# AlexandraLJones/MCBRaT3D

Measured on AMD Instinct MI355X. Metric: photons/sec, higher is better.
Workload: dtype f32/f64

## Files before the change

mcbrat3d_amd/csrc/mcbrat_api.hip:

```cpp
#include <hip/hip_runtime.h>

#include <algorithm>
#include <array>
#include <cfloat>
#include <cmath>
#include <cstdio>
#include <cstdlib>
#include <cstring>
#include <string>
#include <vector>

#include "mcbrat_kernels.hip"
#include "mcbrat_blockwalk.hip"

using namespace mcbrat;

struct mcbrat_ctx {
  int device = 0;
  struct Lane {
    hipStream_t stream = nullptr;
    hipEvent_t ev0 = nullptr, ev1 = nullptr;
    hipEvent_t evDone = nullptr;
    unsigned long long *dCounter = nullptr;
    long long *dSlabs = nullptr;
// ... 33 lines not shown
  uint16_t *dFlyRange = nullptr;
  int flyNbx = 0, flyNby = 0;
  bool flyBuilt = false;
  double flyDepth = 0.0;
  double flightMaxDepth = 0.5;
  uint32_t *dBlockRec = nullptr;
  uint16_t *dBlockOf = nullptr;
  float *dBlockExt = nullptr;
  float *dBlockSsa = nullptr, *dBlockCum = nullptr;
  uint16_t *dBlockPfi = nullptr;
  bool blockOpticsUniform = false;
  int nBlocks = 0;
  int crossThreshold = 8;
  int batchUnits = 0;
  int jumpThreshold = 8;
  bool noSimple3 = false;
  float *dExtB = nullptr, *dCumB = nullptr, *dSsaB = nullptr, *dBgExt = nullptr, *dBgCum = nullptr, *dBgSsa = nullptr;
  uint16_t *dPfiB = nullptr, *dBgPfi = nullptr;
  int nbx = 0, nby = 0, nbz = 0;
  long long nStored = 0;
  double backgroundFraction = 0.0;
  bool bricksBuilt = false;
  int brickMode = 2;
  float *dTables = nullptr;
  int surfNumX = 0, surfNumY = 0;
  double *dSurfX = nullptr, *dSurfY = nullptr;
  float *dSurfRefl = nullptr;
  int surfKind = 0;
  float4 *dSurfBrdf = nullptr;
  double *dVoxelCDF = nullptr;
// ... 392 lines not shown
  return 0;
}

int build_blocks(mcbrat_ctx *c, const std::vector<float> &e, const std::vector<float> &cu, const std::vector<float> &ssa,
                 const std::vector<uint16_t> &pf, int nc) {
  const int nx = c->nx, ny = c->ny, nz = c->nz;
  const size_t nvox = (size_t)nx * ny * nz;
  c->nBlocks = 0;
  if (c->dBlockRec) { (void)hipFree(c->dBlockRec); c->dBlockRec = nullptr; }
  if (c->dBlockOf) { (void)hipFree(c->dBlockOf); c->dBlockOf = nullptr; }
  if (c->dBlockExt) { (void)hipFree(c->dBlockExt); c->dBlockExt = nullptr; }
  if (c->dBlockSsa) { (void)hipFree(c->dBlockSsa); c->dBlockSsa = nullptr; }
  if (c->dBlockCum) { (void)hipFree(c->dBlockCum); c->dBlockCum = nullptr; }
  if (c->dBlockPfi) { (void)hipFree(c->dBlockPfi); c->dBlockPfi = nullptr; }
  c->blockOpticsUniform = false;
  if (nvox > 65536 || nx > 65535 || ny > 65535 || nz > 65535) return 0;
  std::vector<uint16_t> of(nvox);
  std::vector<uint32_t> rec(4 * nvox);
  int32_t nb = 0;
  if (mcbrat_block_decomposition(nx, ny, nz, e.data(), of.data(), rec.data(), &nb) != 0) return 0;
  std::vector<float> blockExt((size_t)nb, 0.0f);
  for (size_t v = 0; v < nvox; ++v) blockExt[of[v]] = e[v];
  if (upload(c, &c->dBlockRec, rec.data(), (size_t)4 * nb) || upload(c, &c->dBlockOf, of.data(), of.size()) ||
      upload(c, &c->dBlockExt, blockExt.data(), blockExt.size())) return 1;
  std::vector<float> bSsa((size_t)nc * nb), bCum((size_t)nc * nb);
  std::vector<uint16_t> bPfi((size_t)nc * nb);
  std::vector<char> seen((size_t)nb, 0);
  bool uniform = true;
  for (size_t v = 0; v < nvox && uniform; ++v) {
    const size_t b = of[v];
    for (int k = 0; k < nc && uniform; ++k) {
      const size_t i = (size_t)k * nvox + v, j = (size_t)k * nb + b;
      if (!seen[b]) { bSsa[j] = ssa[i]; bCum[j] = cu[i]; bPfi[j] = pf[i]; }
      else uniform = std::memcmp(&bSsa[j], &ssa[i], 4) == 0 && std::memcmp(&bCum[j], &cu[i], 4) == 0 && bPfi[j] == pf[i];
    }
    seen[b] = 1;
  }
  if (uniform) {
    if (upload(c, &c->dBlockSsa, bSsa.data(), bSsa.size()) || upload(c, &c->dBlockCum, bCum.data(), bCum.size()) ||
        upload(c, &c->dBlockPfi, bPfi.data(), bPfi.size())) return 1;
    c->blockOpticsUniform = true;
  }
  c->nBlocks = nb;
  return 0;
}

bool use_bricks(const mcbrat_ctx *c) {
  if (!c->bricksBuilt || c->brickMode == 0 || c->nDir > 0 || orders_on(c) || facewalk_on(c)) return false;
  if (c->brickMode == 1) return true;
  const size_t nvox = (size_t)c->nx * c->ny * c->nz;
  return nvox * sizeof(float) >= ((size_t)2 << 30) && c->backgroundFraction >= 0.5;
}

void fill_params(mcbrat_ctx *c, DevParams &p) {
  std::memset(&p, 0, sizeof(p));
  p.nx = c->nx; p.ny = c->ny; p.nz = c->nz; p.nc = c->nc;
  p.xyRegular = c->xyRegular; p.zRegular = c->zRegular;
// ... 315 lines not shown
        MCBRAT_SPEC_CASE(1 | 1 << 2 | 16); MCBRAT_SPEC_CASE(2 | 1 << 2 | 16); MCBRAT_SPEC_CASE(3 | 1 << 2 | 16);
        MCBRAT_SPEC_CASE(1 | 2 << 2 | 16); MCBRAT_SPEC_CASE(2 | 2 << 2 | 16); MCBRAT_SPEC_CASE(3 | 2 << 2 | 16);
#undef MCBRAT_SPEC_CASE
      }
    }
  }
  return trace_ptr<BLOCK, 0, false, DBG>(tbl, emit);
}

template <int BLOCK, bool DBG, int SIMPLE, int OPT>
const void *block_ptr(bool tbl, bool emit) {
  if (tbl) return emit ? (const void *)trace_block_kernel<BLOCK, true, DBG, true, SIMPLE, OPT> : (const void *)trace_block_kernel<BLOCK, true, DBG, false, SIMPLE, OPT>;
  return emit ? (const void *)trace_block_kernel<BLOCK, false, DBG, true, SIMPLE, OPT> : (const void *)trace_block_kernel<BLOCK, false, DBG, false, SIMPLE, OPT>;
}

template <int BLOCK, bool DBG, int OPT = 0>
const void *block_kernel_for(const mcbrat_ctx *c, const DevParams &p, bool tbl) {
  const bool emit = c->srcKind != 0;
  const bool simple = c->xyRegular && c->zRegular && c->nc == 1 && c->surfNumX == 0;
  if constexpr (OPT == 0 && BLOCK != 1024) {
    if (simple && c->ny == 1 && !DBG) return block_ptr<BLOCK, DBG, 2, OPT>(tbl, emit);
  }
  if constexpr (!DBG && (BLOCK == 1024 || BLOCK == 768)) {
    if (!c->xyRegular && !c->zRegular && p.xyNearUniform && p.zNearUniform && c->nc == 1 && c->surfNumX == 0 && !c->noSimple3)
      return block_ptr<BLOCK, DBG, 3, OPT>(tbl, emit);
  }
  return simple ? block_ptr<BLOCK, DBG, 1, OPT>(tbl, emit) : block_ptr<BLOCK, DBG, 0, OPT>(tbl, emit);
}

bool block_walk_applies(const mcbrat_ctx *c, const LaunchPlan &L) {
  return blocks_worth_it(c) && ((L.priv && L.gridLds) || L.blockLite);
}

int launch_block(mcbrat_ctx *c, DevParams &p, const LaunchPlan &L, bool debug, int nBatches) {
// ... 781 lines not shown
             kernel == 2 ? "trace_block_kernel" : "trace_kernel", h[3], kind == DROP_RAY ? "view direction" : "state", state, (unsigned)(h[2] >> 32));
  } else {
    snprintf(buf + at, sizeof(buf) - (size_t)at, "; no photon record (production kernels keep none: trace the same photons with mcbrat_trace_fates)");
  }
  c->dropText = buf;
  return c->dropText.c_str();
}

int mcbrat_set_option(mcbrat_ctx *c, const char *name, int32_t value) {
  if (!c) return 1;
  if (!name) return fail(c, "set_option: no option name");
  const std::string n(name);
  if (n == "jumpThreshold") c->jumpThreshold = std::max(1, std::min(64, (int)value));
  else if (n == "crossThreshold") c->crossThreshold = std::max(1, std::min(64, (int)value));
  else if (n == "batchUnits") c->batchUnits = value != 0;
  else return fail(c, "set_option: unknown option '" + n + "'");
  return 0;
}

int mcbrat_set_surface_description(mcbrat_ctx *c, int32_t numX, int32_t numY, const double *xPosition, const double *yPosition,
                                   const float *reflectance) {
  if (!c) return 1;
  (void)hipSetDevice(c->device);
  if (sync_all(c)) return 1;
  if (numX <= 0 || numY <= 0) { c->surfNumX = c->surfNumY = 0; return 0; }
  if (numX < 2 || numY < 2 || !xPosition || !yPosition || !reflectance)
    return fail(c, "new_SurfaceDescription: position vector(s) are incorrect length.");
  for (int i = 1; i < numX; ++i) if (!(xPosition[i] - xPosition[i - 1] > 0.)) return fail(c, "new_SurfaceDescription: positions must be unique, increasing.");
  for (int i = 1; i < numY; ++i) if (!(yPosition[i] - yPosition[i - 1] > 0.)) return fail(c, "new_SurfaceDescription: positions must be unique, increasing.");
  for (size_t i = 0; i < (size_t)(numX - 1) * (numY - 1); ++i)
// ... 111 lines not shown
  if (e == hipSuccess) e = hipMemcpyAsync(out, dOut, sizeof(uint32_t) * 4 * (size_t)n, hipMemcpyDeviceToHost, st);
  if (e == hipSuccess) e = hipStreamSynchronize(st);
  (void)hipFree(dIn); (void)hipFree(dOut);
  HIP_OK(c, e);
  return 0;
}

int mcbrat_get_walk_mode(const mcbrat_ctx *c) {
  if (!c) return 0;
  int m = (c->layerSkip ? 1 : 0) | (c->blockWalk ? 2 : 0);
  if (c->haveGrid && c->haveOptics) {
    const LaunchPlan L = plan_launch(c, (size_t)tally_layout(flux_run(tally_shape(c))).slabStride);
    m = ((c->layerSkip && !facewalk_on(c)) ? 1 : 0) | (block_walk_applies(c, L) ? 2 : 0) | (L.fly ? 4 : 0) | (c->blockWalk ? 8 : 0) |
        (L.wide ? 16 : 0) | ((L.blockLite && L.optics == 1) ? 32 : 0) | (L.priv ? 64 : 0) | ((L.blockLite && L.optics == 2) ? 128 : 0) |
        (L.cdfTop ? 256 : 0);
  }
  return m;
}

int mcbrat_compute_radiative_transfer(mcbrat_ctx *c, uint64_t seed, uint64_t firstPhotonId, int64_t ppb, int32_t nBatches,
                                      int64_t *numPhotonsProcessed) {
  if (!c) return 1;
  (void)hipSetDevice(c->device);
  if (check_ready(c)) return 1;
  if (ppb < 1 || nBatches < 1) return fail(c, "computeRadiativeTransfer: Didn't process any photons.");
  if (ppb > kMaxPhotonsPerBatch)
    return fail(c, "computeRadiativeTransfer: numPhotonsPerBatch is too large: at most 2^31 - 1 photons per batch fit the tallies.");
  if (ensure_moments(c)) return 1;
  const bool tuneNow = c->autoTune && !c->tuned && (unsigned long long)ppb * (unsigned long long)nBatches >= c->tuneTrialPhotons;
  const bool async = c->asyncOn && !c->countersOn;
// ... 250 lines not shown
```

mcbrat3d_amd/csrc/mcbrat_blockwalk.hip:

```cpp
#include <float.h>

#include "mcbrat_device.h"

namespace mcbrat {

enum : int { BW_DEAD = 0, BW_MOVE = 1, BW_COLLIDE = 2, BW_SURFACE = 3, BW_TOP = 4, BW_CROSS = 5 };

__device__ __forceinline__ int locate_z(const double *ze, int nz, bool regular, double z0, double invDz, double z) {
  if (!regular) return find_cell(ze, nz, z);
  return min(max((int)((z - z0) * invDz), 0), nz - 1);
}
__device__ __forceinline__ int locate_near_uniform(const double *e, int n, double x0, double invCell, double v) {
  int i = min(max((int)((v - x0) * invCell), 0), n - 1);
  const double lo = e[i], hi = e[i + 1];
  i += (v >= hi && i < n - 1) ? 1 : 0;
  i -= (v < lo && i > 0) ? 1 : 0;
  return i;
}

__device__ __forceinline__ long long unwrapped_index(const double *e, int n, double x0, double L, double invL, double x) {
  const double k = floor((x - x0) * invL);
  return (long long)k * n + find_cell(e, n, x - k * L);
}

struct BlockLds {
  size_t slab, cursor, rec, cdf, ext, ssa, cum, pfi, blockOf, tbl, total;
};
__host__ __device__ inline BlockLds block_lds_layout(int nx, int ny, int nz, int nc, size_t slabLen, int nBlocks, size_t tblFloats,
                                                      int optics = 0, bool cdfTop = false) {
  BlockLds L;
  const size_t nvox = (size_t)nx * ny * nz;
  const size_t nB4 = ((size_t)nBlocks + 3) & ~(size_t)3;
  size_t o = sizeof(double) * (size_t)(nx + ny + nz + 3);
  L.slab = o; o += sizeof(long long) * slabLen;
  L.cursor = o; o += 16;
  o = (o + 15) & ~(size_t)15;
  L.rec = o; o += 16 * (size_t)nBlocks;
  L.cdf = o; o += cdfTop ? sizeof(double) * ((size_t)nz + (size_t)ny * nz) : 0;
  L.ext = o; o += optics == 0 ? 4 * nvox : 4 * nB4;
  L.ssa = o; o += optics == 0 ? 4 * nvox * nc : (optics == 2 ? 4 * nB4 * nc : 0);
  L.cum = o; o += nc > 1 ? (optics == 0 ? 4 * nvox * nc : (optics == 2 ? 4 * nB4 * nc : 0)) : 0;
  L.pfi = o; o += optics == 0 ? 2 * ((nvox * nc + 1) & ~(size_t)1) : (optics == 2 ? 2 * nB4 * nc : 0);
  L.blockOf = o; o += 2 * ((nvox + 1) & ~(size_t)1);
  o = (o + 3) & ~(size_t)3;
  L.tbl = o; o += 4 * tblFloats;
  L.total = o;
  return L;
}

template <int BLOCK, bool TBL_LDS, bool DEBUG, bool EMIT, int SIMPLE, int OPT = 0>
__global__ void __launch_bounds__(BLOCK, BLOCK == 1024 ? 4 : (BLOCK > 512 ? BLOCK / 128 : MCBRAT_MIN_WAVES_PER_SIMD))
trace_block_kernel(const DevParams p) {
  constexpr bool NOY = SIMPLE == 2 && !DEBUG;
  constexpr bool NEAR = SIMPLE == 3;
  const bool xyRegular = NEAR ? false : (SIMPLE != 0 ? true : p.xyRegular != 0);
  const bool zRegular = NEAR ? false : (SIMPLE != 0 ? true : p.zRegular != 0);
  const int nc = SIMPLE != 0 ? 1 : p.nc;
  extern __shared__ __align__(16) unsigned char smem_raw[];
#ifdef MCBRAT_POISON
  for (unsigned i = threadIdx.x; i < p.ldsBytes / 4u; i += BLOCK) reinterpret_cast<unsigned *>(smem_raw)[i] = 0xffffffffu;
  __syncthreads();
#endif
  double *s_edge = reinterpret_cast<double *>(smem_raw);
  const int nEdges = p.nx + p.ny + p.nz + 3;
  const int ncol = p.nx * p.ny;
  const int nvox = ncol * p.nz;
  const int slabLen = (int)p.slabStride;
  const int slabsLen = p.unitsWide ? 2 * slabLen : slabLen;
  const bool cdfTop = EMIT && p.cdfTopLds != 0;
  const BlockLds lay = block_lds_layout(p.nx, p.ny, p.nz, nc, (size_t)slabsLen, p.nBlocks, TBL_LDS ? (size_t)p.tblTotalFloats : 0, OPT, cdfTop);
  const int nB4 = (p.nBlocks + 3) & ~3;
  long long *s_slab = reinterpret_cast<long long *>(smem_raw + lay.slab);
  unsigned *s_cursor = reinterpret_cast<unsigned *>(smem_raw + lay.cursor);
  uint4 *s_blockRec = reinterpret_cast<uint4 *>(smem_raw + lay.rec);
  float *s_ext = reinterpret_cast<float *>(smem_raw + lay.ext);
  double *s_cdfLevel = reinterpret_cast<double *>(smem_raw + lay.cdf);
  double *s_cdfRow = s_cdfLevel + p.nz;
  float *s_ssa = reinterpret_cast<float *>(smem_raw + lay.ssa);
  float *s_cum = reinterpret_cast<float *>(smem_raw + lay.cum);
  uint16_t *s_pfi = reinterpret_cast<uint16_t *>(smem_raw + lay.pfi);
  uint16_t *s_blockOf = reinterpret_cast<uint16_t *>(smem_raw + lay.blockOf);
  float *s_tbl = reinterpret_cast<float *>(smem_raw + lay.tbl);
  __shared__ int s_tblOffset[MCBRAT_MAX_COMPONENTS], s_tblNSteps[MCBRAT_MAX_COMPONENTS];
  __shared__ float s_tblInvN[MCBRAT_MAX_COMPONENTS];
  if (threadIdx.x < MCBRAT_MAX_COMPONENTS) {
    s_tblOffset[threadIdx.x] = p.tblOffset[threadIdx.x];
    s_tblNSteps[threadIdx.x] = p.tblNSteps[threadIdx.x];
    s_tblInvN[threadIdx.x] = p.tblInvN[threadIdx.x];
  }
  for (int i = threadIdx.x; i < nEdges; i += BLOCK) s_edge[i] = p.edges[i];
  if (TBL_LDS)
    for (int i = threadIdx.x; i < p.tblTotalFloats; i += BLOCK) s_tbl[i] = p.tables[i];
  for (int i = threadIdx.x; i < slabsLen; i += BLOCK) s_slab[i] = 0;
  if (threadIdx.x == 0) s_cursor[0] = 0;
  for (int i = threadIdx.x; i < p.nBlocks; i += BLOCK) s_blockRec[i] = p.blockRec[i];
  for (int i = threadIdx.x; i < nvox; i += BLOCK) s_blockOf[i] = p.blockOf[i];
  if (OPT == 0) {
    for (int i = threadIdx.x; i < nvox; i += BLOCK) s_ext[i] = p.ext[i];
    for (int i = threadIdx.x; i < nc * nvox; i += BLOCK) { s_ssa[i] = p.ssa[i]; s_pfi[i] = p.pfi[i]; }
    if (nc > 1)
      for (int i = threadIdx.x; i < nc * nvox; i += BLOCK) s_cum[i] = p.cum[i];
  } else {
    for (int i = threadIdx.x; i < p.nBlocks; i += BLOCK) s_ext[i] = p.blockExt[i];
    if (OPT == 2) {
      for (int i = threadIdx.x; i < nc * nB4; i += BLOCK) {
        const int k = i / nB4, b = i - k * nB4;
        if (b < p.nBlocks) { s_ssa[i] = p.blockSsa[k * p.nBlocks + b]; s_pfi[i] = p.blockPfi[k * p.nBlocks + b]; if (nc > 1) s_cum[i] = p.blockCum[k * p.nBlocks + b]; }
      }
    }
  }
// ... 9 lines not shown
  auto extOfCell = [&](int cell) -> float { if constexpr (OPT == 0) return s_ext[cell]; else return s_ext[s_blockOf[cell]]; };
  const float *__restrict__ tbl = TBL_LDS ? s_tbl : p.tables;
  const int offY = p.nx + 1, offZ = p.nx + p.ny + 2;
  const double invDz = (double)p.nz / (p.zMax - p.z0);

  const int lane = threadIdx.x & (kWave - 1);

  unsigned long long unitFirst = 0;
  unsigned unitCount = 0, unitSplit = 0;
  long long *unitSlab = nullptr;

  int state = BW_DEAD;
  unsigned long long moreMask = ~0ull;
  int slabOff = 0;
  uint32_t idLo = 0, idHi = 0, event = 0;
  unsigned long long idP1 = 0;
  double px = 0, py = 0, pz = 0;
  float dx = 0, dy = 0, dz = 1;
  float ivx = 0, ivy = 0, ivz = 0;
  float tnx = 0, tny = 0, tnz = 0, tcur = 0;
  float acc = 0, tau = 0, w = 0, extCur = 0, uX = 0, uY = 0, uZ = 0;
  unsigned rx = 0, ry = 0, rz = 0;
  unsigned spans = 0;
  int nScat = 0, nLegs = 0;
  long long dbgX = 0, dbgY = 0;
  int dbgZ = 0;
  unsigned int cLegs = 0, cCross = 0, cColl = 0, cAbs = 0, cTop = 0, cSurf = 0, cKill = 0, cSurv = 0;
  unsigned long long wIters = 0, wCrossPhases = 0, wCrossLanes = 0, wEventLanes = 0, wLaunchPhases = 0, wSurfPhases = 0;

  auto countCrossings = [&](double x, double y, int kzEnd) {
    const long long ex = unwrapped_index(s_edge, p.nx, p.x0, p.Lx, p.invLx, x);
    const long long ey = unwrapped_index(s_edge + offY, p.ny, p.y0, p.Ly, p.invLy, y);
    cCross += (unsigned)(llabs(ex - dbgX) + llabs(ey - dbgY) + abs(kzEnd - dbgZ));
  };

  auto locX = [&](double xw, bool canLeave, bool force = false) {
    if (p.nx == 1 && !force) return 0;
    if (canLeave) {
// ... 19 lines not shown
  };
  auto inRange = [](int j, unsigned r) { return min(max(j, (int)(r & 0xffffu)), (int)(r >> 16) - 1); };
  const bool legacyNoClamp = (DEBUG || kTestBounds) && (p.legacyTies & 1) != 0, legacyMoveNaN = (DEBUG || kTestBounds) && (p.legacyTies & 2) != 0,
             legacyKeepSpans = (DEBUG || kTestBounds) && (p.legacyTies & 4) != 0;
  auto inRangeX = [&](int j, unsigned r) { return legacyNoClamp ? j : inRange(j, r); };
  const unsigned nx24 = (unsigned)p.nx, ncol24 = (unsigned)ncol;
  auto cellOf = [&](int ix, int iy, int iz) -> int {
    if (NOY) return ix + (int)__umul24(ncol24, (unsigned)iz);
    return ix + (int)__umul24(nx24, (unsigned)(iy + (int)__umul24((unsigned)p.ny, (unsigned)iz)));
  };
  auto enterBlock = [&](int ix, int iy, int iz) {
    const int cell = cellOf(ix, iy, iz);
    const unsigned blk = s_blockOf[cell];
    const uint4 rec = s_blockRec[blk];
    if constexpr (OPT == 0) extCur = s_ext[cell]; else extCur = s_ext[blk];
    rx = rec.x; rz = rec.z;
    if (!NOY) ry = rec.y;
    const int fx = dx >= 0.0f ? (int)(rx >> 16) : (int)(rx & 0xffffu);
    const int fy = NOY ? 0 : (dy >= 0.0f ? (int)(ry >> 16) : (int)(ry & 0xffffu));
    const int fz = dz >= 0.0f ? (int)(rz >> 16) : (int)(rz & 0xffffu);
    spans |= rec.w;
    const float ex = (float)(s_edge[fx] - px), ez = (float)(s_edge[offZ + fz] - pz);
    tnx = ((rec.w & 1u) || ivx == 0.0f) ? FLT_MAX : ex * ivx;
    tny = (NOY || (rec.w & 2u) || ivy == 0.0f) ? FLT_MAX : (float)(s_edge[offY + fy] - py) * ivy;
    tnz = ivz == 0.0f ? FLT_MAX : ez * ivz;
  };

  unsigned nCrossLeg = 0;
  unsigned nBadLane = 0;
  const unsigned maxEvents = (DEBUG || kTestBounds) ? p.maxEvents : kMaxEvents, maxEventsNaN = (DEBUG || kTestBounds) ? p.maxEventsNaN : kMaxEventsNaN,
                 watchdog = (DEBUG || kTestBounds) ? p.watchdog : kWatchdog;
#define MCBRAT_BW_DROP(kind_) do { \
    if constexpr (DEBUG || kTestBounds) record_first_drop(p.bad, (kind_), 2u, idLo, idHi, state, event);   \
    if (DEBUG && p.fates) p.fates[(((unsigned long long)idHi << 32) | idLo) - p.firstPhoton] = mcbrat_fate{3, 0, 0, 0, nScat, nLegs, w}; \
    state = BW_DEAD; \
    nBadLane = count_drop(nBadLane, (kind_));   \
  } while (0)
#ifdef MCBRAT_STAMPS
  __shared__ unsigned long long s_tprev[BLOCK / 64], s_stamp[BLOCK / 64][9];
// ... 20 lines not shown
    moreMask = ~0ull;

    for (;;) {
      bool needLeg = false;
      int ix = 0, iy = 0, iz = 0;

      const unsigned long long mSurf = __ballot(state == BW_SURFACE || state == BW_TOP);
      const unsigned long long mCross = __ballot(state == BW_CROSS);
      const int nBusy = __popcll(__ballot(state == BW_COLLIDE));
      const bool idle = nBusy < p.eventThreshold;
      const bool doSurface = __popcll(mSurf) >= p.surfaceThreshold || idle;
      const bool doCross = __popcll(mCross) >= p.crossThreshold || idle;
      if ((state == BW_SURFACE || state == BW_TOP) && doSurface) {
        const bool top = state == BW_TOP;
        {
          const double xw = px + (double)tcur * (double)dx, yw = py + (double)tcur * (double)dy;
          if (DEBUG) countCrossings(xw, yw, top ? p.nz : -1);
          px = xw;
          if (!NOY) py = yw;
          const int jx = locX(xw, true, true);
          ix = inRange(jx, rx);
          if (ix != jx) {
            const double lo = s_edge[rx & 0xffffu], hi = s_edge[rx >> 16];
            if (px < lo && lo - px > px + p.Lx - hi) px += p.Lx;
            else if (px > hi && px - hi > lo - (px - p.Lx)) px -= p.Lx;
          }
          iy = 0;
          if (!NOY) {
            const int jy = locY(yw, true, true);
            iy = inRange(jy, ry);
            if (iy != jy) {
// ... 8 lines not shown
          if (DEBUG) {
            cTop++;
            if (p.fates) p.fates[(((unsigned long long)idHi << 32) | idLo) - p.firstPhoton] = mcbrat_fate{0, ix + 1, iy + 1, p.nz + 1, nScat, nLegs, w};
          }
          state = BW_DEAD;
        } else {
          pz = p.zSurf;
          iz = 0;
          nScat++;
          if (DEBUG) cSurf++;
          float mu = sqrtf(uX);
          if (!(fabsf(mu) > 2.0f * FLT_MIN)) {
            mu = sqrtf(uZ);
            uint32_t r[4];
            for (uint32_t j = 0; !(fabsf(mu) > 2.0f * FLT_MIN); j++) {
              if ((j & 3u) == 0) philox4x32_10_p1(event, 2u + (j >> 2), idP1, idHi, p.seedLo, p.seedHi, r);
              mu = sqrtf(u01(pick4(r, j & 3u)));
            }
          }
          const float wIn = w;
          if (SIMPLE == 0 && p.surfNumX > 0) w = w * surface_reflectance(p, px, py);
          else w = (float)((double)w * (double)p.albedo);
          if (w <= FLT_MIN) {
            if (DEBUG && p.fates) p.fates[(((unsigned long long)idHi << 32) | idLo) - p.firstPhoton] = mcbrat_fate{1, ix + 1, iy + 1, 1, nScat, nLegs, wIn};
            state = BW_DEAD;
          } else {
            const float sinTheta = sqrtf(1.0f - mu * mu);
            float cphi, sphi;
            sincos_2pi(uY, cphi, sphi);
            dx = sinTheta * cphi; dy = sinTheta * sphi; dz = mu;
            needLeg = true;
// ... 14 lines not shown
      if (want != 0ull) {
        const int nWant = __popcll(want);
        const unsigned rank = __builtin_amdgcn_mbcnt_hi((unsigned)(want >> 32), __builtin_amdgcn_mbcnt_lo((unsigned)want, 0u));
        unsigned base = 0;
        if (lane == 0) base = atomicAdd(&s_cursor[0], (unsigned)nWant);
        base = (unsigned)__shfl((int)base, 0);
        const unsigned k = base + rank;
        const bool valid = k < unitCount;
        const unsigned long long myIdx = unitFirst + k;
        const unsigned long long mValid = __ballot(valid);
        if (__builtin_amdgcn_inverse_ballot_w64(want)) {
          if (valid) {
            const unsigned long long id = p.firstPhoton + myIdx;
            idLo = (uint32_t)id; idHi = (uint32_t)(id >> 32);
            idP1 = philox_p1(idLo);
            event = 0; nScat = 0; nLegs = 0;
            slabOff = k < unitSplit ? 0 : slabLen;
            uint32_t r[4];
            philox4x32_10_p1(0u, 0u, idP1, idHi, p.seedLo, p.seedHi, r);
            double lx, ly, lz;
            if (!EMIT) {
              lz = 0.0;
              if (p.solarKind == 0) {
                lx = (double)u01(r[0]);
                ly = (double)u01(r[1]);
                dx = p.dir0[0]; dy = p.dir0[1]; dz = p.dir0[2];
              } else {
                solar_launch(p, r[0], r[1], r[2], r[3], [&](uint32_t b) {
                  uint32_t o[4];
                  philox4x32_10_p1(0u, b, idP1, idHi, p.seedLo, p.seedHi, o);
// ... 62 lines not shown
              const double t = (lz - p.z0) * (double)p.nz;
              const double fl = floor(t);
              iz = min((int)fl, p.nz - 1);
              pz = s_edge[offZ + iz] + (t - fl) * (s_edge[offZ + iz + 1] - s_edge[offZ + iz]);
            }
            if (EMIT && p.lwFlag && pz > 0.0)
              atomicAdd(reinterpret_cast<unsigned long long *>(s_slab + slabOff + 2 * ncol + (ix + p.nx * (iy + p.ny * iz))), to_fixed(-1.0));
            needLeg = true;
          }
        }
        moreMask &= ~want | mValid;
      }
      STAMP(0);
      if (state == BW_COLLIDE) {
        if (dz == dz || legacyMoveNaN) {
          const double s = (double)(tcur + div_fast(tau - acc, extCur));
          px = px + s * (double)dx;
          if (!NOY) py = py + s * (double)dy;
          pz = pz + s * (double)dz;
        }
        {
          const double xw = px, yw = py;
          iz = NEAR ? locate_near_uniform(s_edge + offZ, p.nz, p.z0, invDz, pz) : locate_z(s_edge + offZ, p.nz, zRegular, p.z0, invDz, pz);
          ix = locX(xw, (spans & 1u) != 0);
          iy = locY(yw, (spans & 2u) != 0);
        }
        int cell = cellOf(ix, iy, iz);
        nScat++;
        if (DEBUG) cColl++;
        int c = 0;
        if (nc > 1) {
          for (int k = 0; k < nc - 1; k++)
            if (uZ >= cumAt(k, cell)) c = k + 1;
        }
        float ssa = ssaAt(c, cell);
        int pfEntry = pfiAt(c, cell);
        if (ssa <= 0.0f && extOfCell(cell) != extCur) {
          ix = inRange(ix, rx); iz = inRange(iz, rz);
          if (!NOY) iy = inRange(iy, ry);
          cell = cellOf(ix, iy, iz);
// ... 3 lines not shown
              if (uZ >= cumAt(k, cell)) c = k + 1;
          }
          ssa = ssaAt(c, cell);
          pfEntry = pfiAt(c, cell);
        }
        if (DEBUG) countCrossings(px, py, iz);
        if (ssa < 1.0f) {
          atomicAdd(reinterpret_cast<unsigned long long *>(s_slab + slabOff + 2 * ncol + cell), weight_to_fixed(w * (1.0f - ssa)));
          w = w * ssa;
          if (DEBUG) cAbs++;
        }
        if (p.useRR && w < 0.5f) {
          float uR = uZ;
          if (nc != 1) {
            uint32_t r1[4];
            philox4x32_10_p1(event, 1u, idP1, idHi, p.seedLo, p.seedHi, r1);
            uR = u01(r1[1]);
          }
          if (uR >= w) { w = 0.0f; if (DEBUG) cKill++; }
          else { w = 1.0f; if (DEBUG) cSurv++; }
        }
        STAMP(2);
        if (w <= FLT_MIN) {
          if (DEBUG && p.fates) p.fates[(((unsigned long long)idHi << 32) | idLo) - p.firstPhoton] = mcbrat_fate{2, ix + 1, iy + 1, iz + 1, nScat, nLegs, 0.0f};
          state = BW_DEAD;
        } else {
          const int n = s_tblNSteps[c];
          const float *t = tbl + s_tblOffset[c] + (TBL_LDS ? (long long)__umul24((unsigned)pfEntry, (unsigned)n) : (long long)pfEntry * n);
          const int ai = (int)(uX * (float)n) + 1;
          float ang;
          if (ai < n) {
// ... 32 lines not shown
      }
      STAMP(4);
      if (needLeg && event >= maxEventsNaN) {
        if (event >= maxEvents || !(dz == dz || w < 1.0f)) { needLeg = false; MCBRAT_BW_DROP(event >= maxEvents ? DROP_LEGS : DROP_NAN_LEGS); }
      }
      if (needLeg) {
        event++;
        nLegs++;
        if (DEBUG) {
          cLegs++;
          dbgX = unwrapped_index(s_edge, p.nx, p.x0, p.Lx, p.invLx, px);
          dbgY = unwrapped_index(s_edge + offY, p.ny, p.y0, p.Ly, p.invLy, py);
          dbgZ = iz;
        }
        uint32_t r[4];
        philox4x32_10_p1(event, 0u, idP1, idHi, p.seedLo, p.seedHi, r);
#ifdef MCBRAT_PRECISE_MATH
        tau = -logf(fmaxf(FLT_MIN, u01(r[0])));
#else
        tau = -0.693147182f * __builtin_amdgcn_logf(fmaxf(FLT_MIN, u01(r[0])));
#endif
        uX = u01(r[1]); uY = u01(r[2]); uZ = u01(r[3]);
        acc = 0.0f; tcur = 0.0f;
        ivx = fabsf(dx) >= 2.0f * FLT_MIN ? rcp_fast(dx) : 0.0f;
        ivy = (!NOY && fabsf(dy) >= 2.0f * FLT_MIN) ? rcp_fast(dy) : 0.0f;
        ivz = fabsf(dz) >= 2.0f * FLT_MIN ? rcp_fast(dz) : 0.0f;
        spans = 0;
        nCrossLeg = 0u;
        enterBlock(ix, iy, iz);
        state = BW_MOVE;
      }
      STAMP(6);
      if (state == BW_CROSS && doCross) {
        const bool yLtX = !NOY && tny < tnx;
        const float m2 = yLtX ? tny : tnx;
        const bool isZ = tnz < m2;
        const double xw = px + (double)tcur * (double)dx, yw = py + (double)tcur * (double)dy, zw = pz + (double)tcur * (double)dz;
        int jx, jy, jz;
        if (isZ) {
          jz = dz >= 0.0f ? (int)(rz >> 16) : (int)(rz & 0xffffu) - 1;
          jx = inRangeX(locX(xw, (spans & 1u) != 0), rx);
          jy = NOY ? 0 : inRangeX(locY(yw, (spans & 2u) != 0), ry);
        } else if (yLtX) {
          jy = dy >= 0.0f ? (int)(ry >> 16) : (int)(ry & 0xffffu) - 1;
          if (jy >= p.ny) { jy = 0; py -= p.Ly; if (DEBUG) dbgY -= p.ny; }
          else if (jy < 0) { jy = p.ny - 1; py += p.Ly; if (DEBUG) dbgY += p.ny; }
          jx = inRangeX(locX(xw, (spans & 1u) != 0), rx);
          jz = inRangeX(NEAR ? locate_near_uniform(s_edge + offZ, p.nz, p.z0, invDz, zw) : locate_z(s_edge + offZ, p.nz, zRegular, p.z0, invDz, zw), rz);
        } else {
          jx = dx >= 0.0f ? (int)(rx >> 16) : (int)(rx & 0xffffu) - 1;
          if (jx >= p.nx) { jx = 0; px -= p.Lx; if (DEBUG) dbgX -= p.nx; }
          else if (jx < 0) { jx = p.nx - 1; px += p.Lx; if (DEBUG) dbgX += p.nx; }
          jy = NOY ? 0 : inRangeX(locY(yw, (spans & 2u) != 0), ry);
          jz = inRangeX(NEAR ? locate_near_uniform(s_edge + offZ, p.nz, p.z0, invDz, zw) : locate_z(s_edge + offZ, p.nz, zRegular, p.z0, invDz, zw), rz);
        }
        if (!legacyKeepSpans) spans = 0;
        enterBlock(jx, jy, jz);
        state = BW_MOVE;
        if (++nCrossLeg > watchdog) MCBRAT_BW_DROP(DROP_CROSSINGS);
      }
      STAMP(1);
      if ((__ballot(state != BW_DEAD) | moreMask) == 0ull) break;

#ifdef MCBRAT_STUCK_PROBE
      if (DEBUG && p.traceBuf && wIters > 3000000ull) {
        const unsigned long long live = __ballot(state != BW_DEAD);
        if (live != 0ull && lane == __ffsll((long long)live) - 1) {
          const unsigned long long r = wIters - 3000001ull;
          if (r < 64ull) {
            double *t = p.traceBuf + 20 * r;
            t[0] = 777; t[1] = state; t[2] = tcur; t[3] = tnx; t[4] = tny; t[5] = tnz; t[6] = (double)rx; t[7] = (double)ry; t[8] = (double)rz;
// ... 62 lines not shown
```

mcbrat3d_amd/csrc/mcbrat_kernels.hip:

```cpp
#include <float.h>

#include "mcbrat_device.h"
#include "mcbrat_brdf.h"
#include "mcbrat_layout.h"

#ifdef MCBRAT_STAMPS
#define STAMP(i) do { if (DEBUG && p.counters) { const unsigned long long t_ = clock64(); \
    if (lane == __ffsll((long long)__ballot(1)) - 1) { s_stamp[threadIdx.x >> 6][i] += t_ - s_tprev[threadIdx.x >> 6]; s_tprev[threadIdx.x >> 6] = t_; } } } while (0)
#elif defined(MCBRAT_MARKS)
#define STAMP(i) asm volatile("; @@mark " #i)
#else
#define STAMP(i) do { } while (0)
#endif

namespace mcbrat {

constexpr unsigned kChunk = 256;
#ifndef MCBRAT_FLY_MIN_BRICKS
#define MCBRAT_FLY_MIN_BRICKS 8.0f
#endif
constexpr float kFlyMinBricks = MCBRAT_FLY_MIN_BRICKS;
constexpr int kWalkCap = 256;

#ifndef MCBRAT_MIN_WAVES_PER_SIMD
// ... 33 lines not shown
__device__ __forceinline__ unsigned long long philox_p1(uint32_t c2) { return (unsigned long long)0xCD9E8D57u * c2; }
__device__ __forceinline__ void philox4x32_10_p1(uint32_t c0, uint32_t c1, unsigned long long p1, uint32_t c3, uint32_t k0,
                                                 uint32_t k1, uint32_t (&out)[4]) {
  const unsigned long long p0 = (unsigned long long)0xD2511F53u * c0;
  uint32_t d0 = xor3((uint32_t)(p1 >> 32), c1, k0), d1 = (uint32_t)p1, d2 = xor3((uint32_t)(p0 >> 32), c3, k1), d3 = (uint32_t)p0;
#pragma unroll
  for (int i = 1; i < 10; i++) {
    k0 += 0x9E3779B9u;
    k1 += 0xBB67AE85u;
    const unsigned long long q0 = (unsigned long long)0xD2511F53u * d0;
    const unsigned long long q1 = (unsigned long long)0xCD9E8D57u * d2;
    d0 = xor3((uint32_t)(q1 >> 32), d1, k0);
    d1 = (uint32_t)q1;
    d2 = xor3((uint32_t)(q0 >> 32), d3, k1);
    d3 = (uint32_t)q0;
  }
  out[0] = d0; out[1] = d1; out[2] = d2; out[3] = d3;
}

__device__ __forceinline__ float u01(uint32_t u) { return (float)u * 2.3283064365386963e-10f; }

#ifdef MCBRAT_PRECISE_MATH
__device__ __forceinline__ float rcp_fast(float x) { return 1.0f / x; }
__device__ __forceinline__ float div_fast(float a, float b) { return a / b; }
#else
__device__ __forceinline__ float rcp_fast(float x) { return __builtin_amdgcn_rcpf(x); }
__device__ __forceinline__ float div_fast(float a, float b) { return a * __builtin_amdgcn_rcpf(b); }
#endif

__device__ __forceinline__ float cos_0_pi(float x) {
// ... 1962 lines not shown
```

mcbrat3d_amd/integrator.py:

```python
import ctypes as C

import numpy as np

from ._capi import Counters, FATE_DTYPE, McbratError, check, lib, ptr

defaultMinInverseTableSize = 9001
defaultMinForwardTableSize = 9001
defaultHybridPhaseFunWidth, maxHybridPhaseFunWidth = 7.0, 30.0
defaultZetaMin = 0.3

_SOLAR_ARGS = {"Directional": ("solarMu", "solarAzimuth"), "RandomAzimuth": ("solarMu",), "Flux": (),
               "Spotlight": ("solarMu", "solarAzimuth", "solarX", "solarY")}
_SOLAR_SETTERS = {"Directional": "mcbrat_set_source_solar", "RandomAzimuth": "mcbrat_set_source_random_azimuth",
                  "Flux": "mcbrat_set_source_flux", "Spotlight": "mcbrat_set_source_spotlight"}


class RandomNumberSequence:

    def __init__(self, seed=10, firstPhotonId=0):
        self.seed = int(seed) & 0xFFFFFFFFFFFFFFFF
        self.nextPhotonId = int(firstPhotonId)


SIDE_FLUX_NAMES = ("sideFluxXPlus", "sideFluxXMinus", "sideFluxYPlus", "sideFluxYMinus")
# ... 329 lines not shown
    def setTuning(self, blocksPerCU=-1, eventThreshold=0, maxBatchesInFlight=-1, privateTallies=-1, blockSize=-1,
                  launchThreshold=0, surfaceThreshold=0, brickLayout=-1, layerSkip=-1, blockWalk=-1):
        self._check(self._lib.mcbrat_set_tuning(self._ctx, blocksPerCU, eventThreshold, maxBatchesInFlight,
                                                privateTallies, blockSize, launchThreshold, surfaceThreshold, brickLayout))
        if layerSkip >= 0 or blockWalk >= 0:
            self._check(self._lib.mcbrat_set_walk_options(self._ctx, int(layerSkip), int(blockWalk)))

    def setOption(self, **options):
        for name, value in options.items():
            self._check(self._lib.mcbrat_set_option(self._ctx, name.encode(), int(value)))

    def walkMode(self):
        m = int(self._lib.mcbrat_get_walk_mode(self._ctx))
        return {"layerSkip": bool(m & 1), "blockWalk": bool(m & 2), "clearAirFlight": bool(m & 4),
                "privateTallies": bool(m & 64), "widePlan": bool(m & 16), "opticsInGlobalMemory": bool(m & 32),
                "opticsPerBlock": bool(m & 128), "emissionCdfTopInLds": bool(m & 256)}

    def badPhotons(self):
        return self.counters()["badPhotons"]

    def firstDrop(self):
        msg = self._lib.mcbrat_first_drop(self._ctx)
        return msg.decode() if msg else ""

    def eventThreshold(self):
        return int(self._lib.mcbrat_get_event_threshold(self._ctx))

    def setAsync(self, enable=True, _chained=False):
        if enable and getattr(self, "_shares_moments", False) and not _chained:
            raise McbratError("setAsync: this integrator accumulates into a moment array it shares with other integrators "
                              "(SpectralRun); their finish kernels are only ordered in synchronous mode, or by chainAfter")
# ... 213 lines not shown
```

Measured before the change: 5.767 billion.

## Specialize block-walk kernel for span-free blocks and hoist per-photon Philox and reciprocal work

Adds a NOSPAN template variant of the block-walk kernel. It is selected when no block spans the periodic X/Y seam, which compiles out the span tracking and span tests. It also precomputes per-block reciprocal extinctions in LDS so the collision distance uses a multiply instead of a division. The first Philox round for the leg random draw is hoisted per photon. Position updates switch to explicit FMA, which can change rounding slightly, and the extra LDS array adds pressure on shared memory.

```diff
diff --git a/mcbrat3d_amd/csrc/mcbrat_api.hip b/mcbrat3d_amd/csrc/mcbrat_api.hip
--- a/mcbrat3d_amd/csrc/mcbrat_api.hip
+++ b/mcbrat3d_amd/csrc/mcbrat_api.hip
@@ -71,6 +71,8 @@
   int crossThreshold = 8;
   int batchUnits = 0;
   int jumpThreshold = 8;
+  bool blockSpansX = true, blockSpansY = true;
+  int blockSpanKernel = 0;
   bool noSimple3 = false;
   float *dExtB = nullptr, *dCumB = nullptr, *dSsaB = nullptr, *dBgExt = nullptr, *dBgCum = nullptr, *dBgSsa = nullptr;
   uint16_t *dPfiB = nullptr, *dBgPfi = nullptr;
@@ -493,6 +495,7 @@
   if (c->dBlockCum) { (void)hipFree(c->dBlockCum); c->dBlockCum = nullptr; }
   if (c->dBlockPfi) { (void)hipFree(c->dBlockPfi); c->dBlockPfi = nullptr; }
   c->blockOpticsUniform = false;
+  c->blockSpansX = c->blockSpansY = true;
   if (nvox > 65536 || nx > 65535 || ny > 65535 || nz > 65535) return 0;
   std::vector<uint16_t> of(nvox);
   std::vector<uint32_t> rec(4 * nvox);
@@ -520,6 +523,9 @@
         upload(c, &c->dBlockPfi, bPfi.data(), bPfi.size())) return 1;
     c->blockOpticsUniform = true;
   }
+  bool sx = false, sy = false;
+  for (int32_t b = 0; b < nb; ++b) { sx = sx || (rec[4 * (size_t)b + 3] & 1u); sy = sy || (rec[4 * (size_t)b + 3] & 2u); }
+  c->blockSpansX = sx; c->blockSpansY = sy;
   c->nBlocks = nb;
   return 0;
 }
@@ -865,10 +871,22 @@
   return emit ? (const void *)trace_block_kernel<BLOCK, false, DBG, true, SIMPLE, OPT> : (const void *)trace_block_kernel<BLOCK, false, DBG, false, SIMPLE, OPT>;
 }
 
+bool nospan_kernel(const mcbrat_ctx *c) {
+  const bool simple = c->xyRegular && c->zRegular && c->nc == 1 && c->surfNumX == 0;
+  if (!simple || c->srcKind != 0 || c->blockSpanKernel != 0) return false;
+  return !c->blockSpansX && (c->ny == 1 || !c->blockSpansY);
+}
+
 template <int BLOCK, bool DBG, int OPT = 0>
 const void *block_kernel_for(const mcbrat_ctx *c, const DevParams &p, bool tbl) {
   const bool emit = c->srcKind != 0;
   const bool simple = c->xyRegular && c->zRegular && c->nc == 1 && c->surfNumX == 0;
+  if constexpr (OPT == 0 && BLOCK == 768 && !DBG) {
+    if (nospan_kernel(c)) {
+      if (c->ny == 1) return tbl ? (const void *)trace_block_kernel<768, true, false, false, 2, 0, true> : (const void *)trace_block_kernel<768, false, false, false, 2, 0, true>;
+      return tbl ? (const void *)trace_block_kernel<768, true, false, false, 1, 0, true> : (const void *)trace_block_kernel<768, false, false, false, 1, 0, true>;
+    }
+  }
   if constexpr (OPT == 0 && BLOCK != 1024) {
     if (simple && c->ny == 1 && !DBG) return block_ptr<BLOCK, DBG, 2, OPT>(tbl, emit);
   }
@@ -1680,6 +1698,7 @@
   if (n == "jumpThreshold") c->jumpThreshold = std::max(1, std::min(64, (int)value));
   else if (n == "crossThreshold") c->crossThreshold = std::max(1, std::min(64, (int)value));
   else if (n == "batchUnits") c->batchUnits = value != 0;
+  else if (n == "blockSpanKernel") c->blockSpanKernel = value != 0;
   else return fail(c, "set_option: unknown option '" + n + "'");
   return 0;
 }
@@ -1821,6 +1840,7 @@
     m = ((c->layerSkip && !facewalk_on(c)) ? 1 : 0) | (block_walk_applies(c, L) ? 2 : 0) | (L.fly ? 4 : 0) | (c->blockWalk ? 8 : 0) |
         (L.wide ? 16 : 0) | ((L.blockLite && L.optics == 1) ? 32 : 0) | (L.priv ? 64 : 0) | ((L.blockLite && L.optics == 2) ? 128 : 0) |
         (L.cdfTop ? 256 : 0);
+    if (block_walk_applies(c, L) && !L.wide && (c->blockSize == 0 || c->blockSize == 768) && nospan_kernel(c)) m |= 512;
   }
   return m;
 }
diff --git a/mcbrat3d_amd/csrc/mcbrat_blockwalk.hip b/mcbrat3d_amd/csrc/mcbrat_blockwalk.hip
--- a/mcbrat3d_amd/csrc/mcbrat_blockwalk.hip
+++ b/mcbrat3d_amd/csrc/mcbrat_blockwalk.hip
@@ -24,7 +24,7 @@
 }
 
 struct BlockLds {
-  size_t slab, cursor, rec, cdf, ext, ssa, cum, pfi, blockOf, tbl, total;
+  size_t slab, cursor, rec, invExt, cdf, ext, ssa, cum, pfi, blockOf, tbl, total;
 };
 __host__ __device__ inline BlockLds block_lds_layout(int nx, int ny, int nz, int nc, size_t slabLen, int nBlocks, size_t tblFloats,
                                                       int optics = 0, bool cdfTop = false) {
@@ -36,6 +36,7 @@
   L.cursor = o; o += 16;
   o = (o + 15) & ~(size_t)15;
   L.rec = o; o += 16 * (size_t)nBlocks;
+  L.invExt = o; o += 4 * nB4;
   L.cdf = o; o += cdfTop ? sizeof(double) * ((size_t)nz + (size_t)ny * nz) : 0;
   L.ext = o; o += optics == 0 ? 4 * nvox : 4 * nB4;
   L.ssa = o; o += optics == 0 ? 4 * nvox * nc : (optics == 2 ? 4 * nB4 * nc : 0);
@@ -48,10 +49,11 @@
   return L;
 }
 
-template <int BLOCK, bool TBL_LDS, bool DEBUG, bool EMIT, int SIMPLE, int OPT = 0>
+template <int BLOCK, bool TBL_LDS, bool DEBUG, bool EMIT, int SIMPLE, int OPT = 0, bool NOSPAN = false>
 __global__ void __launch_bounds__(BLOCK, BLOCK == 1024 ? 4 : (BLOCK > 512 ? BLOCK / 128 : MCBRAT_MIN_WAVES_PER_SIMD))
 trace_block_kernel(const DevParams p) {
   constexpr bool NOY = SIMPLE == 2 && !DEBUG;
+  constexpr bool HOIST = !DEBUG && (BLOCK != 768 || (SIMPLE == 2 && !EMIT));
   constexpr bool NEAR = SIMPLE == 3;
   const bool xyRegular = NEAR ? false : (SIMPLE != 0 ? true : p.xyRegular != 0);
   const bool zRegular = NEAR ? false : (SIMPLE != 0 ? true : p.zRegular != 0);
@@ -73,6 +75,7 @@
   long long *s_slab = reinterpret_cast<long long *>(smem_raw + lay.slab);
   unsigned *s_cursor = reinterpret_cast<unsigned *>(smem_raw + lay.cursor);
   uint4 *s_blockRec = reinterpret_cast<uint4 *>(smem_raw + lay.rec);
+  float *s_invExt = reinterpret_cast<float *>(smem_raw + lay.invExt);
   float *s_ext = reinterpret_cast<float *>(smem_raw + lay.ext);
   double *s_cdfLevel = reinterpret_cast<double *>(smem_raw + lay.cdf);
   double *s_cdfRow = s_cdfLevel + p.nz;
@@ -93,7 +96,7 @@
     for (int i = threadIdx.x; i < p.tblTotalFloats; i += BLOCK) s_tbl[i] = p.tables[i];
   for (int i = threadIdx.x; i < slabsLen; i += BLOCK) s_slab[i] = 0;
   if (threadIdx.x == 0) s_cursor[0] = 0;
-  for (int i = threadIdx.x; i < p.nBlocks; i += BLOCK) s_blockRec[i] = p.blockRec[i];
+  for (int i = threadIdx.x; i < p.nBlocks; i += BLOCK) { s_blockRec[i] = p.blockRec[i]; s_invExt[i] = rcp_fast(p.blockExt[i]); }
   for (int i = threadIdx.x; i < nvox; i += BLOCK) s_blockOf[i] = p.blockOf[i];
   if (OPT == 0) {
     for (int i = threadIdx.x; i < nvox; i += BLOCK) s_ext[i] = p.ext[i];
@@ -133,14 +136,19 @@
   unsigned long long moreMask = ~0ull;
   int slabOff = 0;
   uint32_t idLo = 0, idHi = 0, event = 0;
+  unsigned long long legQ0 = 0;
+  uint32_t legD1 = 0;
   unsigned long long idP1 = 0;
+  auto photonP1 = [&]() { if constexpr (HOIST) return philox_p1(idLo); else return idP1; };
   double px = 0, py = 0, pz = 0;
   float dx = 0, dy = 0, dz = 1;
   float ivx = 0, ivy = 0, ivz = 0;
   float tnx = 0, tny = 0, tnz = 0, tcur = 0;
-  float acc = 0, tau = 0, w = 0, extCur = 0, uX = 0, uY = 0, uZ = 0;
+  float acc = 0, tau = 0, w = 0, extCur = 0, invExtCur = 0, uX = 0, uY = 0, uZ = 0;
   unsigned rx = 0, ry = 0, rz = 0;
   unsigned spans = 0;
+  auto spanX = [&]() { return !NOSPAN && (spans & 1u) != 0; };
+  auto spanY = [&]() { return !NOSPAN && (spans & 2u) != 0; };
   int nScat = 0, nLegs = 0;
   long long dbgX = 0, dbgY = 0;
   int dbgZ = 0;
@@ -190,15 +198,16 @@
     const unsigned blk = s_blockOf[cell];
     const uint4 rec = s_blockRec[blk];
     if constexpr (OPT == 0) extCur = s_ext[cell]; else extCur = s_ext[blk];
+    if constexpr (HOIST) invExtCur = s_invExt[blk];
     rx = rec.x; rz = rec.z;
     if (!NOY) ry = rec.y;
     const int fx = dx >= 0.0f ? (int)(rx >> 16) : (int)(rx & 0xffffu);
     const int fy = NOY ? 0 : (dy >= 0.0f ? (int)(ry >> 16) : (int)(ry & 0xffffu));
     const int fz = dz >= 0.0f ? (int)(rz >> 16) : (int)(rz & 0xffffu);
-    spans |= rec.w;
+    if constexpr (!NOSPAN) spans |= rec.w;
     const float ex = (float)(s_edge[fx] - px), ez = (float)(s_edge[offZ + fz] - pz);
-    tnx = ((rec.w & 1u) || ivx == 0.0f) ? FLT_MAX : ex * ivx;
-    tny = (NOY || (rec.w & 2u) || ivy == 0.0f) ? FLT_MAX : (float)(s_edge[offY + fy] - py) * ivy;
+    tnx = ((!NOSPAN && (rec.w & 1u)) || ivx == 0.0f) ? FLT_MAX : ex * ivx;
+    tny = (NOY || (!NOSPAN && (rec.w & 2u)) || ivy == 0.0f) ? FLT_MAX : (float)(s_edge[offY + fy] - py) * ivy;
     tnz = ivz == 0.0f ? FLT_MAX : ez * ivz;
   };
 
@@ -249,7 +258,7 @@
       if ((state == BW_SURFACE || state == BW_TOP) && doSurface) {
         const bool top = state == BW_TOP;
         {
-          const double xw = px + (double)tcur * (double)dx, yw = py + (double)tcur * (double)dy;
+          const double xw = __fma_rn((double)tcur, (double)dx, px), yw = __fma_rn((double)tcur, (double)dy, py);
           if (DEBUG) countCrossings(xw, yw, top ? p.nz : -1);
           px = xw;
           if (!NOY) py = yw;
@@ -288,7 +297,7 @@
             mu = sqrtf(uZ);
             uint32_t r[4];
             for (uint32_t j = 0; !(fabsf(mu) > 2.0f * FLT_MIN); j++) {
-              if ((j & 3u) == 0) philox4x32_10_p1(event, 2u + (j >> 2), idP1, idHi, p.seedLo, p.seedHi, r);
+              if ((j & 3u) == 0) philox4x32_10_p1(event, 2u + (j >> 2), photonP1(), idHi, p.seedLo, p.seedHi, r);
               mu = sqrtf(u01(pick4(r, j & 3u)));
             }
           }
@@ -333,6 +342,7 @@
             const unsigned long long id = p.firstPhoton + myIdx;
             idLo = (uint32_t)id; idHi = (uint32_t)(id >> 32);
             idP1 = philox_p1(idLo);
+            if constexpr (HOIST) { legQ0 = philox_leg_q0(idP1, p.seedLo); legD1 = (uint32_t)idP1; }
             event = 0; nScat = 0; nLegs = 0;
             slabOff = k < unitSplit ? 0 : slabLen;
             uint32_t r[4];
@@ -425,16 +435,20 @@
       STAMP(0);
       if (state == BW_COLLIDE) {
         if (dz == dz || legacyMoveNaN) {
+#ifdef MCBRAT_PRECISE_MATH
           const double s = (double)(tcur + div_fast(tau - acc, extCur));
-          px = px + s * (double)dx;
-          if (!NOY) py = py + s * (double)dy;
-          pz = pz + s * (double)dz;
+#else
+          const double s = (double)(tcur + (HOIST ? (tau - acc) * invExtCur : div_fast(tau - acc, extCur)));
+#endif
+          px = __fma_rn(s, (double)dx, px);
+          if (!NOY) py = __fma_rn(s, (double)dy, py);
+          pz = __fma_rn(s, (double)dz, pz);
         }
         {
           const double xw = px, yw = py;
           iz = NEAR ? locate_near_uniform(s_edge + offZ, p.nz, p.z0, invDz, pz) : locate_z(s_edge + offZ, p.nz, zRegular, p.z0, invDz, pz);
-          ix = locX(xw, (spans & 1u) != 0);
-          iy = locY(yw, (spans & 2u) != 0);
+          ix = locX(xw, spanX());
+          iy = locY(yw, spanY());
         }
         int cell = cellOf(ix, iy, iz);
         nScat++;
@@ -468,7 +482,7 @@
           float uR = uZ;
           if (nc != 1) {
             uint32_t r1[4];
-            philox4x32_10_p1(event, 1u, idP1, idHi, p.seedLo, p.seedHi, r1);
+            philox4x32_10_p1(event, 1u, photonP1(), idHi, p.seedLo, p.seedHi, r1);
             uR = u01(r1[1]);
           }
           if (uR >= w) { w = 0.0f; if (DEBUG) cKill++; }
@@ -531,7 +545,8 @@
           dbgZ = iz;
         }
         uint32_t r[4];
-        philox4x32_10_p1(event, 0u, idP1, idHi, p.seedLo, p.seedHi, r);
+        if constexpr (HOIST) philox4x32_10_leg(event, legQ0, legD1, idHi, p.seedLo, p.seedHi, r);
+        else philox4x32_10_p1(event, 0u, idP1, idHi, p.seedLo, p.seedHi, r);
 #ifdef MCBRAT_PRECISE_MATH
         tau = -logf(fmaxf(FLT_MIN, u01(r[0])));
 #else
@@ -542,7 +557,7 @@
         ivx = fabsf(dx) >= 2.0f * FLT_MIN ? rcp_fast(dx) : 0.0f;
         ivy = (!NOY && fabsf(dy) >= 2.0f * FLT_MIN) ? rcp_fast(dy) : 0.0f;
         ivz = fabsf(dz) >= 2.0f * FLT_MIN ? rcp_fast(dz) : 0.0f;
-        spans = 0;
+        if constexpr (!NOSPAN) spans = 0;
         nCrossLeg = 0u;
         enterBlock(ix, iy, iz);
         state = BW_MOVE;
@@ -552,26 +567,26 @@
         const bool yLtX = !NOY && tny < tnx;
         const float m2 = yLtX ? tny : tnx;
         const bool isZ = tnz < m2;
-        const double xw = px + (double)tcur * (double)dx, yw = py + (double)tcur * (double)dy, zw = pz + (double)tcur * (double)dz;
+        const double xw = __fma_rn((double)tcur, (double)dx, px), yw = __fma_rn((double)tcur, (double)dy, py), zw = __fma_rn((double)tcur, (double)dz, pz);
         int jx, jy, jz;
         if (isZ) {
           jz = dz >= 0.0f ? (int)(rz >> 16) : (int)(rz & 0xffffu) - 1;
-          jx = inRangeX(locX(xw, (spans & 1u) != 0), rx);
-          jy = NOY ? 0 : inRangeX(locY(yw, (spans & 2u) != 0), ry);
+          jx = inRangeX(locX(xw, spanX()), rx);
+          jy = NOY ? 0 : inRangeX(locY(yw, spanY()), ry);
         } else if (yLtX) {
           jy = dy >= 0.0f ? (int)(ry >> 16) : (int)(ry & 0xffffu) - 1;
           if (jy >= p.ny) { jy = 0; py -= p.Ly; if (DEBUG) dbgY -= p.ny; }
           else if (jy < 0) { jy = p.ny - 1; py += p.Ly; if (DEBUG) dbgY += p.ny; }
-          jx = inRangeX(locX(xw, (spans & 1u) != 0), rx);
+          jx = inRangeX(locX(xw, spanX()), rx);
           jz = inRangeX(NEAR ? locate_near_uniform(s_edge + offZ, p.nz, p.z0, invDz, zw) : locate_z(s_edge + offZ, p.nz, zRegular, p.z0, invDz, zw), rz);
         } else {
           jx = dx >= 0.0f ? (int)(rx >> 16) : (int)(rx & 0xffffu) - 1;
           if (jx >= p.nx) { jx = 0; px -= p.Lx; if (DEBUG) dbgX -= p.nx; }
           else if (jx < 0) { jx = p.nx - 1; px += p.Lx; if (DEBUG) dbgX += p.nx; }
-          jy = NOY ? 0 : inRangeX(locY(yw, (spans & 2u) != 0), ry);
+          jy = NOY ? 0 : inRangeX(locY(yw, spanY()), ry);
           jz = inRangeX(NEAR ? locate_near_uniform(s_edge + offZ, p.nz, p.z0, invDz, zw) : locate_z(s_edge + offZ, p.nz, zRegular, p.z0, invDz, zw), rz);
         }
-        if (!legacyKeepSpans) spans = 0;
+        if (!NOSPAN && !legacyKeepSpans) spans = 0;
         enterBlock(jx, jy, jz);
         state = BW_MOVE;
         if (++nCrossLeg > watchdog) MCBRAT_BW_DROP(DROP_CROSSINGS);
diff --git a/mcbrat3d_amd/csrc/mcbrat_kernels.hip b/mcbrat3d_amd/csrc/mcbrat_kernels.hip
--- a/mcbrat3d_amd/csrc/mcbrat_kernels.hip
+++ b/mcbrat3d_amd/csrc/mcbrat_kernels.hip
@@ -71,6 +71,31 @@
     d1 = (uint32_t)q1;
     d2 = xor3((uint32_t)(q0 >> 32), d3, k1);
     d3 = (uint32_t)q0;
+  }
+  out[0] = d0; out[1] = d1; out[2] = d2; out[3] = d3;
+}
+
+__device__ __forceinline__ unsigned long long philox_leg_q0(unsigned long long p1, uint32_t k0) {
+  return (unsigned long long)0xD2511F53u * ((uint32_t)(p1 >> 32) ^ k0);
+}
+__device__ __forceinline__ void philox4x32_10_leg(uint32_t c0, unsigned long long q0, uint32_t p1Lo, uint32_t c3, uint32_t k0,
+                                                  uint32_t k1, uint32_t (&out)[4]) {
+  const unsigned long long p0 = (unsigned long long)0xD2511F53u * c0;
+  uint32_t e2 = xor3((uint32_t)(p0 >> 32), c3, k1), e3 = (uint32_t)p0;
+  k0 += 0x9E3779B9u;
+  k1 += 0xBB67AE85u;
+  const unsigned long long r1 = (unsigned long long)0xCD9E8D57u * e2;
+  uint32_t d0 = xor3((uint32_t)(r1 >> 32), p1Lo, k0), d1 = (uint32_t)r1, d2 = xor3((uint32_t)(q0 >> 32), e3, k1), d3 = (uint32_t)q0;
+#pragma unroll
+  for (int i = 2; i < 10; i++) {
+    k0 += 0x9E3779B9u;
+    k1 += 0xBB67AE85u;
+    const unsigned long long q0i = (unsigned long long)0xD2511F53u * d0;
+    const unsigned long long q1i = (unsigned long long)0xCD9E8D57u * d2;
+    d0 = xor3((uint32_t)(q1i >> 32), d1, k0);
+    d1 = (uint32_t)q1i;
+    d2 = xor3((uint32_t)(q0i >> 32), d3, k1);
+    d3 = (uint32_t)q0i;
   }
   out[0] = d0; out[1] = d1; out[2] = d2; out[3] = d3;
 }
diff --git a/mcbrat3d_amd/integrator.py b/mcbrat3d_amd/integrator.py
--- a/mcbrat3d_amd/integrator.py
+++ b/mcbrat3d_amd/integrator.py
@@ -367,7 +367,8 @@
         m = int(self._lib.mcbrat_get_walk_mode(self._ctx))
         return {"layerSkip": bool(m & 1), "blockWalk": bool(m & 2), "clearAirFlight": bool(m & 4),
                 "privateTallies": bool(m & 64), "widePlan": bool(m & 16), "opticsInGlobalMemory": bool(m & 32),
-                "opticsPerBlock": bool(m & 128), "emissionCdfTopInLds": bool(m & 256)}
+                "opticsPerBlock": bool(m & 128), "emissionCdfTopInLds": bool(m & 256),
+                "foldsCompiledOut": bool(m & 512)}
 
     def badPhotons(self):
         return self.counters()["badPhotons"]
```

Measured after the change: 6.013 billion (median of 6 runs). +4.3%, better.
